# Gabrielcb/DaliID

Hardware: AMD Instinct MI355X
Metric: images/sec (train step) (higher is better)
Workload: dtype bf16; 1 GPU; configs[1]: ResNet-50 ReID bf16 256x128, PK batch 16x16=256 per GPU, center+proxy heads, Adam, EMA; global_batch=256, per_gpu_batch=256, parallelism=dp1

## Files before the change

### daliid_amd/csrc/conv.hip

```cpp
#include "gemm_tile.h"
#include "kernels.h"
#include "../../include/daliid_debug.h"
#include <cstdlib>
#include <type_traits>
#include <vector>
#include <string>
#include <cstdio>

namespace dali {

__device__ __forceinline__ void decode_pixel(const GatherGeom& g, int p, int& n, int& ho, int& wo) {
    if (g.lhw >= 0 && g.lw >= 0) {
        n = p >> g.lhw;
        const int rem = p & ((1 << g.lhw) - 1);
        ho = rem >> g.lw;
        wo = rem & ((1 << g.lw) - 1);
    } else {
        const int hw = g.Hout * g.Wout;
        n = p / hw;
        const int rem = p - n * hw;
        ho = rem / g.Wout;
        wo = rem - ho * g.Wout;
    }
}
// ... 1007 lines not shown
            for (int j = 0; j < FN; ++j) {
                const bf16x8_t fb = *reinterpret_cast<const bf16x8_t*>(patch + (boff[j] ^ (uint32_t)(h << 5)));
#pragma unroll
                for (int i = 0; i < FM; ++i) acc[i][j] = __builtin_amdgcn_mfma_f32_16x16x32_bf16(fa[i], fb, acc[i][j], 0, 0, 0);
            }
        }
        asm volatile("s_waitcnt lgkmcnt(0)" ::: "memory");
        __builtin_amdgcn_s_barrier();
    }
    conv_epilogue_g<TM, TN, FM, FN, 4, NT, EPI>(a, acc, 0, tn, smem, 0, wn);
}

}
#include "fused1x1.h"
namespace dali {

__device__ __forceinline__ int wg_swz(int row) { return (row & 3) | (((row >> 3) & 1) << 2); }

typedef short s16x4_t __attribute__((ext_vector_type(4)));

__device__ __forceinline__ int tr_frag_off(int chunk32, int lane, int half) {
    const int row = 8 * (lane >> 4) + ((lane & 15) >> 2) + 4 * half;
    return row * 128 + ((chunk32 ^ wg_swz(row)) << 4) + 4 * (lane & 3);
}
typedef short s16x8_t __attribute__((ext_vector_type(8)));
__device__ __forceinline__ bf16x8_t tr_frag(const uint16_t* tile, int chunk32, int lane) {
    typedef __attribute__((address_space(3))) s16x4_t* lds_ptr_t;
    const s16x4_t a = __builtin_amdgcn_ds_read_tr16_b64_v4i16((lds_ptr_t)(tile + tr_frag_off(chunk32, lane, 0)));
    const s16x4_t b = __builtin_amdgcn_ds_read_tr16_b64_v4i16((lds_ptr_t)(tile + tr_frag_off(chunk32, lane, 1)));
    return __builtin_bit_cast(bf16x8_t, s16x8_t{a[0], a[1], a[2], a[3], b[0], b[1], b[2], b[3]});
}

struct TrPair { s16x4_t lo, hi; };
__device__ __forceinline__ s16x4_t ds_read_tr_raw(const uint16_t* p) {
    typedef __attribute__((address_space(3))) const uint16_t* lds_cptr_t;
    const uint32_t addr = (uint32_t)(uintptr_t)(lds_cptr_t)p;
    s16x4_t v;
    asm volatile("ds_read_b64_tr_b16 %0, %1" : "=v"(v) : "v"(addr));
    return v;
}
__device__ __forceinline__ TrPair tr_frag_raw(const uint16_t* tile, int chunk32, int lane) {
    return TrPair{ds_read_tr_raw(tile + tr_frag_off(chunk32, lane, 0)), ds_read_tr_raw(tile + tr_frag_off(chunk32, lane, 1))};
}
__device__ __forceinline__ bf16x8_t tr_join(const TrPair& t) {
    return __builtin_bit_cast(bf16x8_t, s16x8_t{t.lo[0], t.lo[1], t.lo[2], t.lo[3], t.hi[0], t.hi[1], t.hi[2], t.hi[3]});
}
template <int N>
__device__ __forceinline__ void tr_settle(TrPair& a, TrPair& b, TrPair& c, TrPair& d) {
    static_assert(N == 0 || N == 8 || N == 10 || N == 16 || N == 18, "lgkmcnt immediates used by the callers");
    asm volatile("s_waitcnt lgkmcnt(%8)" : "+v"(a.lo), "+v"(a.hi), "+v"(b.lo), "+v"(b.hi), "+v"(c.lo), "+v"(c.hi), "+v"(d.lo), "+v"(d.hi) : "n"(N > 15 ? 15 : N));
}

__device__ __forceinline__ void tr_settle_all(TrPair& a) { asm volatile("s_waitcnt lgkmcnt(0)" : "+v"(a.lo), "+v"(a.hi)); }

template <int FM, int FN>
__device__ __forceinline__ void store_slab_tiles(float* slab, const f32x4_t (&acc)[FM][FN], int m_first, int n_first, int Cm, int Ntot, int lane) {
    const int mr = m_first + (lane >> 4) * 4, nc = n_first + (lane & 15);
    if (m_first + 16 * FM <= Cm && n_first + 16 * FN <= Ntot) {
        float* row = slab + (size_t)mr * Ntot + nc;
#pragma unroll
        for (int i = 0; i < FM; ++i)
#pragma unroll
            for (int rr = 0; rr < 4; ++rr) {
                float* p = row + (size_t)(i * 16 + rr) * Ntot;
#pragma unroll
                for (int j = 0; j < FN; ++j) p[j * 16] = acc[i][j][rr];
            }
        return;
    }
#pragma unroll
    for (int i = 0; i < FM; ++i)
#pragma unroll
        for (int j = 0; j < FN; ++j) {
            const int n = nc + j * 16;
#pragma unroll
            for (int rr = 0; rr < 4; ++rr) {
                const int m = mr + i * 16 + rr;
                if (m < Cm && n < Ntot) slab[(size_t)m * Ntot + n] = acc[i][j][rr];
            }
        }
}


struct WGradWork {
    int ks, tm, tn, p_begin, p_end, ksteps;
    __device__ __forceinline__ void set(const WGradArgs& a, unsigned item, int tiles_m, int tiles_n) {
        const unsigned tiles = tiles_m * tiles_n;
        ks = item / tiles;
        const int tile = item - ks * tiles;
        tm = tile / tiles_n; tn = tile - tm * tiles_n;
        p_begin = ks * a.pix_per_split;
        p_end = min(a.P, p_begin + a.pix_per_split);
        ksteps = (p_end > p_begin) ? (p_end - p_begin + 31) >> 5 : 0;
    }
    __device__ __forceinline__ bool map_xcd(const WGradArgs& a, int tiles_m, int tiles_n) {
        const int work = tiles_m * tiles_n * a.splits, per_xcd = (work + 7) >> 3;
        const int item = (blockIdx.x & 7) * per_xcd + (blockIdx.x >> 3);
        if ((int)(blockIdx.x >> 3) >= per_xcd || item >= work) return false;
        set(a, item, tiles_m, tiles_n);
        return true;
    }
};

struct WGradRsrc { __amdgpu_buffer_rsrc_t y, x; };
__device__ __forceinline__ WGradRsrc wgrad_rsrc(const WGradArgs& a) {
    const GatherGeom& g = a.g;
// ... 227 lines not shown
        }
    };

    f32x4_t acc[4][4];
#pragma unroll
    for (int i = 0; i < 4; ++i)
#pragma unroll
        for (int j = 0; j < 4; ++j) acc[i][j] = f32x4_t{0.f, 0.f, 0.f, 0.f};
    const bool do_cs = COLSUM && tn == 0 && wn == 0;
    f32x4_t cs[4];
#pragma unroll
    for (int i = 0; i < 4; ++i) cs[i] = f32x4_t{0.f, 0.f, 0.f, 0.f};
    typedef short ones_vec_t __attribute__((ext_vector_type(8)));
    const bf16x8_t ones = __builtin_bit_cast(bf16x8_t, ones_vec_t{0x3F80, 0x3F80, 0x3F80, 0x3F80, 0x3F80, 0x3F80, 0x3F80, 0x3F80});

    if (ksteps > 0) {
        issue(0, 0);
        if (ksteps > 1) issue(1, 1);
        if (ksteps > 1) dma_wait<4>(); else dma_wait<0>();
        __builtin_amdgcn_s_barrier();
        conv_stamp(a, 1);
        int st_cur = 0, st_nxt2 = 2;
        for (int kt = 0; kt < ksteps; ++kt) {
            if (kt + 2 < ksteps) issue(kt + 2, st_nxt2);
            const uint16_t* sa = smem + st_cur * 2 * TILE;
            const uint16_t* sb = sa + TILE;
            bf16x8_t fa[4];
            wgrad_tr_kstep(sa, wm * 4, sb, wn * 4, lane, acc, fa);
            if constexpr (COLSUM) if (do_cs) {
#pragma unroll
                for (int i = 0; i < 4; ++i) cs[i] = __builtin_amdgcn_mfma_f32_16x16x32_bf16(fa[i], ones, cs[i], 0, 0, 0);
            }
            if (kt + 2 < ksteps) dma_wait<4>(); else dma_wait<0>();
            __builtin_amdgcn_s_barrier();
            st_cur = (st_cur == 2) ? 0 : st_cur + 1;
            st_nxt2 = (st_nxt2 == 2) ? 0 : st_nxt2 + 1;
        }
    }
    conv_stamp(a, 2);
    float* slab = a.partial + (size_t)ks * a.Cm * a.Ntot;
    store_slab_tiles<4, 4>(slab, acc, m0 + wm * 64, n0 + wn * 64, a.Cm, a.Ntot, lane);
    if constexpr (COLSUM) if (do_cs && (lane & 15) == 0) {
#pragma unroll
        for (int i = 0; i < 4; ++i)
#pragma unroll
            for (int rr = 0; rr < 4; ++rr) {
                const int m = m0 + wm * 64 + i * 16 + (lane >> 4) * 4 + rr;
                if (m < a.Cm) a.colsum[(size_t)ks * a.Cm + m] = cs[i][rr];
            }
    }
    conv_stamp_stores(a);
}

__device__ __forceinline__ int halo_swz(int row) { return ((row >> 1) & 1) | (((row >> 3) & 1) << 1); }
constexpr int W3_A_ELEMS = 32 * 128, W3_B_ELEMS = 16 * 512, W3_STAGE = W3_A_ELEMS + W3_B_ELEMS;

template <int NSTAGE>
__global__ __launch_bounds__(512) void igemm_wgrad3x3_kernel(WGradArgs a, int tiles_m, int tiles_n) {
    extern __shared__ __attribute__((aligned(16))) uint16_t smem[];
    const int tid = threadIdx.x, lane = tid & 63;
    const int wave = __builtin_amdgcn_readfirstlane(tid >> 6);
    const int wm = wave >> 2, wn = wave & 3;
    WGradWork wk;
    if (!wk.map_xcd(a, tiles_m, tiles_n)) return;
    const int ks = wk.ks, m0 = wk.tm * 128, ci0 = wk.tn * 64;
    conv_stamp(a, 0);
    const bool m_active = m0 + wm * 64 < a.Cm;
    const GatherGeom g = a.g;
    const int W = g.Wout, H = g.Hout, Cin = g.Ck, lw = g.lw, lhw = g.lhw;
    const int RW = 32 >> lw, HC = W + 2, HP = (RW + 2) * HC;
    const WGradRsrc rs = wgrad_rsrc(a);

    const int r_in = lane >> 4, ps = lane & 15;
    const int c16 = ((((ps >> 1) ^ wg_swz(4 * wave + r_in)) << 1) | (ps & 1));
    const int am = m0 + c16 * 8;
    const bool a_ok = am < a.Cm;
    int hb_hr[2], hb_off[2];
    bool hb_ok[2];
#pragma unroll
    for (int i = 0; i < 2; ++i) {
        const int hp = 8 * (wave + 8 * i) + (lane >> 3);
        const int lc = (lane & 7) ^ (halo_swz(hp) << 1);
        const int hr = hp / HC, hc = hp - hr * HC;
        hb_hr[i] = hr;
        hb_ok[i] = hp < HP && (unsigned)(hc - 1) < (unsigned)W && ci0 + lc * 8 < Cin;
        hb_off[i] = ((hc - 1) * Cin + ci0 + lc * 8) * 2;
    }
    const int p_begin = wk.p_begin, p_end = wk.p_end, ksteps = wk.ksteps;

    auto issue = [&](int kt, int stage) {
        uint16_t* sa = smem + stage * W3_STAGE;
        uint16_t* sb = sa + W3_A_ELEMS;
        const int p0 = p_begin + kt * 32;
        const int p = p0 + 4 * wave + r_in;
        const uint32_t oa = (p < p_end && a_ok) ? (uint32_t)(p * a.Cm + am) * 2u : DMA_OOB;
        __builtin_amdgcn_raw_ptr_buffer_load_lds(rs.y, (lds_void_ptr)(sa + wave * 512), 16, oa, 0, 0, 0);
        const int n = p0 >> lhw, h_base = (p0 & ((1 << lhw) - 1)) >> lw;
        const int row_bytes = W * Cin * 2;
        const int img_base = (int)((long long)n * g.img_pitch * 2);
#pragma unroll
        for (int i = 0; i < 2; ++i) {
            const int h = h_base - 1 + hb_hr[i];
            const bool ok = hb_ok[i] && (unsigned)h < (unsigned)H && p0 < p_end;
            const uint32_t ob = ok ? (uint32_t)(img_base + h * row_bytes + hb_off[i]) : DMA_OOB;
            __builtin_amdgcn_raw_ptr_buffer_load_lds(rs.x, (lds_void_ptr)(sb + (wave + 8 * i) * 512), 16, ob, 0, 0, 0);
        }
    };

    f32x4_t acc[9][4];
#pragma unroll
    for (int t = 0; t < 9; ++t)
#pragma unroll
        for (int i = 0; i < 4; ++i) acc[t][i] = f32x4_t{0.f, 0.f, 0.f, 0.f};
    const int gq = lane >> 4, q = (lane & 15) >> 2, pp = lane & 3;
    const int hrow_base = ((8 * gq) >> lw) * HC + ((8 * gq) & (W - 1)) + q;
    int boff0[9], boff1[9];
#pragma unroll
    for (int r = 0; r < 3; ++r)
#pragma unroll
        for (int s2 = 0; s2 < 3; ++s2) {
            const int row0 = hrow_base + r * HC + s2, row1 = row0 + 4;
            boff0[r * 3 + s2] = row0 * 64 + ((wn ^ halo_swz(row0)) << 4) + 4 * pp;
            boff1[r * 3 + s2] = row1 * 64 + ((wn ^ halo_swz(row1)) << 4) + 4 * pp;
        }
    auto load_b = [&](const uint16_t* sb, int t) -> TrPair { return TrPair{ds_read_tr_raw(sb + boff0[t]), ds_read_tr_raw(sb + boff1[t])}; };

    constexpr int AHEAD = NSTAGE - 1;
    auto wait_inflight = [&](int n) {
        if (n <= 0) dma_wait<0>();
        else if (n == 1) dma_wait<3>();
        else if (n == 2) dma_wait<6>();
        else if (n == 3) dma_wait<9>();
        else dma_wait<12>();
    };
    static_assert(AHEAD >= 1 && AHEAD <= 5, "ring depth");
    if (ksteps > 0) {
        int issued = 0;
        for (; issued < AHEAD && issued < ksteps; ++issued) issue(issued, issued);
        wait_inflight(issued - 1 > 4 ? 4 : issued - 1);
        __builtin_amdgcn_s_barrier();
        conv_stamp(a, 1);
        int st_cur = 0, st_fill = AHEAD % NSTAGE;
        for (int kt = 0; kt < ksteps; ++kt) {
            if (kt + AHEAD < ksteps) issue(kt + AHEAD, st_fill);
            const uint16_t* sa = smem + st_cur * W3_STAGE;
            const uint16_t* sb = sa + W3_A_ELEMS;
            if (m_active) {
            TrPair ra[4], rb[9];
#pragma unroll
            for (int i = 0; i < 4; ++i) ra[i] = tr_frag_raw(sa, wm * 4 + i, lane);
#pragma unroll
            for (int t = 0; t < 9; ++t) rb[t] = load_b(sb, t);
            tr_settle<18>(ra[0], ra[1], ra[2], ra[3]);
            tr_settle<10>(rb[0], rb[1], rb[2], rb[3]);
            bf16x8_t fa[4];
#pragma unroll
            for (int i = 0; i < 4; ++i) fa[i] = tr_join(ra[i]);
#pragma unroll
            for (int t = 0; t < 4; ++t) {
                const bf16x8_t fb = tr_join(rb[t]);
#pragma unroll
                for (int i = 0; i < 4; ++i) acc[t][i] = __builtin_amdgcn_mfma_f32_16x16x32_bf16(fa[i], fb, acc[t][i], 0, 0, 0);
            }
            __builtin_amdgcn_sched_barrier(0);
            tr_settle<0>(rb[4], rb[5], rb[6], rb[7]);
            tr_settle_all(rb[8]);
#pragma unroll
            for (int t = 4; t < 9; ++t) {
                const bf16x8_t fb = tr_join(rb[t]);
#pragma unroll
                for (int i = 0; i < 4; ++i) acc[t][i] = __builtin_amdgcn_mfma_f32_16x16x32_bf16(fa[i], fb, acc[t][i], 0, 0, 0);
            }
            }
            const int left = ksteps - 1 - kt;
            const int keep = (left < AHEAD ? left : AHEAD) - 1;
            wait_inflight(keep > 4 ? 4 : keep);
            __builtin_amdgcn_s_barrier();
            st_cur = (st_cur == NSTAGE - 1) ? 0 : st_cur + 1;
            st_fill = (st_fill == NSTAGE - 1) ? 0 : st_fill + 1;
        }
    }
    conv_stamp(a, 2);
    float* slab = a.partial + (size_t)ks * a.Cm * a.Ntot;
    if (m_active) {
        float* row = slab + (size_t)(m0 + wm * 64 + (lane >> 4) * 4) * a.Ntot + ci0 + wn * 16 + (lane & 15);
#pragma unroll
        for (int i = 0; i < 4; ++i)
#pragma unroll
            for (int rr = 0; rr < 4; ++rr) {
                float* p = row + (size_t)(i * 16 + rr) * a.Ntot;
#pragma unroll
                for (int t = 0; t < 9; ++t) p[t * Cin] = acc[t][i][rr];
            }
    }
    conv_stamp_stores(a);
}

template <int WM, int WN, int NSTAGE, bool COLSUM = false>
__global__ __launch_bounds__(WM * WN * 64, 4) void igemm_wgrad_wg_kernel(WGradArgs a, int tiles_m, int tiles_n) {
    constexpr int TM = 64 * WM, TN = 64 * WN, NW = WM * WN;
    using Gather = WGradGather<TM / 128, (TM + TN) / 128, NW>;
    constexpr int IMG = Gather::IMG, NIMG_A = Gather::NIMG_A, STAGE = Gather::STAGE, NDMA = Gather::NDMA;
    constexpr int AHEAD = NSTAGE - 1;
    static_assert(TM % 128 == 0 && TN % 128 == 0, "unsupported wave grid");
    extern __shared__ __attribute__((aligned(16))) uint16_t smem[];
    const int tid = threadIdx.x, lane = tid & 63;
    const int wave = __builtin_amdgcn_readfirstlane(tid >> 6);
    const int wm = wave / WN, wn = wave % WN;
    WGradWork wk;
    if (!wk.map_xcd(a, tiles_m, tiles_n)) return;
    const int m0 = wk.tm * TM, n0 = wk.tn * TN, ksteps = wk.ksteps;
    const Gather gather(a, wave, m0, n0, wk.p_begin, wk.p_end, lane);

    const bool do_cs = COLSUM && wn == 0;
    int cs_turn = wk.tn;
    f32x4_t cs = f32x4_t{0.f, 0.f, 0.f, 0.f};
    typedef unsigned sel_vec_t __attribute__((ext_vector_type(4)));
    const int cs_col = (lane & 15) >> 2;
    f32x4_t acc[4][4];
#pragma unroll
    for (int i = 0; i < 4; ++i)
#pragma unroll
        for (int j = 0; j < 4; ++j) acc[i][j] = f32x4_t{0.f, 0.f, 0.f, 0.f};
    if (ksteps > 0) {
        int issued = 0;
        for (; issued < AHEAD && issued < ksteps; ++issued) gather.issue(issued, smem + issued * STAGE);
        if (issued == 1) dma_wait<0>();
        else if (issued == 2) dma_wait<NDMA>();
        else dma_wait<2 * NDMA>();
        __builtin_amdgcn_s_barrier();
        int st_cur = 0, st_fill = AHEAD % NSTAGE;
        for (int kt = 0; kt < ksteps; ++kt) {
            if (kt + AHEAD < ksteps) gather.issue(kt + AHEAD, smem + st_fill * STAGE);
            const uint16_t* sa = smem + st_cur * STAGE + (wm >> 1) * IMG;
            const uint16_t* sb = smem + st_cur * STAGE + (NIMG_A + (wn >> 1)) * IMG;
            bf16x8_t fa[4];
            wgrad_tr_kstep(sa, (wm & 1) * 4, sb, (wn & 1) * 4, lane, acc, fa);
            if constexpr (COLSUM) if (do_cs) {
                if (cs_turn == 0) {
                    int opaque;
// ... 374 lines not shown
    using Shape = RingShape<64, WM, WN, 4, 4, NSTAGE>;
    return {name, kfn(&igemm_conv_k64s_kernel<WM, WN, NP, NSTAGE, 4, 4, MODE, SRC2>), Shape::NT + NP * 64, Shape::LDS_BYTES, Shape::TM, Shape::TN, GRID_XCD};
}

static const GemmKernel
    CONV128_BN{"CONV128_BN", kfn(&igemm_conv_kernel<128, 128, true>), 256, REG128_LDS, 128, 128, GRID_XCD},
    CONV128{"CONV128", kfn(&igemm_conv_kernel<128, 128, false>), 256, REG128_LDS, 128, 128, GRID_XCD},
    DMA128 = ring_kernel<32, 2, 2, 4, 4, 3, 4, true, Epi::CONV>("DMA128"),
    DMA128_LIN = ring_kernel<32, 2, 2, 4, 4, 3, 4, true, Epi::LIN>("DMA128_LIN"),
    DMA128_FUSED = ring_kernel<32, 2, 2, 4, 4, 3, 3, true, Epi::FUSED>("DMA128_FUSED"),
    DMA128_CLS = ring_kernel<32, 2, 2, 4, 4, 3, 4, true, Epi::PARITY>("DMA128_CLS"),
    DMA128_SRC2 = ring_kernel<32, 2, 2, 4, 4, 3, 4, true, Epi::CONV, true>("DMA128_SRC2"),
    CONV64_BN{"CONV64_BN", kfn(&igemm_conv_kernel<64, 256, true>), 256, REG64_LDS, 64, 256, GRID_XCD},
    CONV64{"CONV64", kfn(&igemm_conv_kernel<64, 256, false>), 256, REG64_LDS, 64, 256, GRID_XCD},
    DMA64 = ring_kernel<32, 2, 2, 2, 8, 3, 2, true, Epi::GENERAL>("DMA64"),
    DMA64_LEAN = ring_kernel<32, 2, 2, 2, 8, 3, 2, true, Epi::FUSED_LEAN>("DMA64_LEAN"),
    DMA64_SRC2 = ring_kernel<32, 2, 2, 2, 8, 3, 2, true, Epi::GENERAL, true>("DMA64_SRC2"),
    K64S64 = k64s_kernel<1, 4, 4, 2, Epi::GENERAL>("K64S64"),
    HALO64{"HALO64", kfn(&igemm_conv_halo64_kernel<3, Epi::GENERAL>), 512, HALO64_LDS, 64, 256, GRID_HALO},
    HALO64_LEAN{"HALO64_LEAN", kfn(&igemm_conv_halo64_kernel<3, Epi::FUSED_LEAN>), 512, HALO64_LDS, 64, 256, GRID_HALO},
    WG128 = ring_kernel<32, 2, 4, 4, 4, 3, 4, false, Epi::CONV>("WG128"),
    WG128_LIN = ring_kernel<32, 2, 4, 4, 4, 3, 4, false, Epi::LIN>("WG128_LIN"),
    WG128_FUSED = ring_kernel<32, 2, 4, 4, 4, 3, 4, false, Epi::FUSED>("WG128_FUSED"),
    WG128_CLS = ring_kernel<32, 2, 4, 4, 4, 3, 4, false, Epi::PARITY>("WG128_CLS"),
    WG256 = ring_kernel<32, 4, 4, 4, 4, 4, 4, false, Epi::GENERAL>("WG256"),
    K64S = k64s_kernel<2, 4, 8, 3, Epi::CONV>("K64S"),
    K64S_LIN = k64s_kernel<2, 4, 8, 3, Epi::LIN>("K64S_LIN"),
    K64S_LEAN = k64s_kernel<2, 4, 8, 3, Epi::FUSED_LEAN>("K64S_LEAN"),
    K64S_SRC2 = k64s_kernel<2, 4, 8, 3, Epi::CONV, true>("K64S_SRC2"),
    K64 = ring_kernel<64, 4, 4, 4, 4, 2, 4, true, Epi::CONV>("K64"),
    K64_LIN = ring_kernel<64, 4, 4, 4, 4, 2, 4, true, Epi::LIN>("K64_LIN"),
    K64_FUSED = ring_kernel<64, 4, 4, 4, 4, 2, 4, true, Epi::FUSED>("K64_FUSED"),
    K64_CLS = ring_kernel<64, 4, 4, 4, 4, 2, 4, true, Epi::PARITY>("K64_CLS"),
    K64_SRC2 = ring_kernel<64, 4, 4, 4, 4, 2, 4, true, Epi::CONV, true>("K64_SRC2"),
    K64_FUSED_SRC2 = ring_kernel<64, 4, 4, 4, 4, 2, 4, true, Epi::FUSED, true>("K64_FUSED_SRC2"),
    K64_320 = ring_kernel<64, 4, 4, 4, 5, 2, 4, true, Epi::LIN>("K64_320");

template <int RB, bool RES, bool OM, bool BITS, bool SRC2 = false>
static GemmKernel f1_kernel() {
    static char name[32];
    snprintf(name, sizeof name, "F1_RB%d%s%s%s%s", RB, RES ? "_RES" : "", OM ? "_MASK" : "", BITS ? "_BITS" : "", SRC2 ? "_SRC2" : "");
    return {name, kfn(&fused1x1_persist_kernel<3, RB, RES, OM, BITS, SRC2>), (F1_NC + F1_NP + F1_NR) * 64, f1_lds_bytes(3, RB, RB == 2 ? 128 : F1_KMAX),
            F1_TM, F1_TN, GRID_CUS, 0, RB};
}
static const GemmKernel F1[2][2][2][2] = {
    {{{f1_kernel<2, false, false, false, true>(), f1_kernel<2, false, false, true>()}, {f1_kernel<2, false, true, false>(), f1_kernel<2, false, true, true>()}},
     {{f1_kernel<2, true, false, false>(), f1_kernel<2, true, false, true>()}, {f1_kernel<2, true, true, false>(), f1_kernel<2, true, true, true>()}}},
    {{{f1_kernel<1, false, false, false, true>(), f1_kernel<1, false, false, true>()}, {f1_kernel<1, false, true, false>(), f1_kernel<1, false, true, true>()}},
     {{f1_kernel<1, true, false, false>(), f1_kernel<1, true, false, true>()}, {f1_kernel<1, true, true, false>(), f1_kernel<1, true, true, true>()}}}};

static const GemmKernel
    WG_BN{"WG_BN", kfn(&igemm_wgrad_kernel<true>), 256, 0, 128, 128, GRID_SPLITS},
    WG_PLAIN{"WG_PLAIN", kfn(&igemm_wgrad_kernel<false>), 256, 0, 128, 128, GRID_SPLITS},
    WG_3X3{"WG_3X3", kfn(&igemm_wgrad3x3_kernel<3>), 512, 3 * W3_STAGE * 2, 128, 9 * 64, GRID_SPLITS8, 256};
static const GemmKernel WG_DMA[2] = {
    {"WG_DMA", kfn(&igemm_wgrad_dma_kernel<false>), 256, 0, 128, 128, GRID_SPLITS8},
    {"WG_DMA_COLSUM", kfn(&igemm_wgrad_dma_kernel<true>), 256, 0, 128, 128, GRID_SPLITS8}};
static const GemmKernel WG_WG[2] = {
    {"WG_WG", kfn(&igemm_wgrad_wg_kernel<2, 4, 3>), 512, ring_lds(128, 256, 32, 3), 128, 256, GRID_SPLITS8, 512},
    {"WG_WG_COLSUM", kfn(&igemm_wgrad_wg_kernel<2, 4, 3, true>), 512, ring_lds(128, 256, 32, 3), 128, 256, GRID_SPLITS8, 512}};
static const GemmKernel WG_P[2][2] = {
    {{"WG_P", kfn(&igemm_wgrad_p_kernel<2, 4, 4, 4, 8, 6>), 1024, ring_lds(128, 256, 32, 6), 128, 256, GRID_SPLITS8, 256},
     {"WG_P_COLSUM", kfn(&igemm_wgrad_p_kernel<2, 4, 4, 4, 8, 6, true>), 1024, ring_lds(128, 256, 32, 6), 128, 256, GRID_SPLITS8, 256}},
    {{"WG_P_FLAT", kfn(&igemm_wgrad_p_kernel<1, 4, 8, 4, 4, 6>), 512, ring_lds(128, 256, 32, 6), 128, 256, GRID_SPLITS8, 256},
     {"WG_P_FLAT_COLSUM", kfn(&igemm_wgrad_p_kernel<1, 4, 8, 4, 4, 6, true>), 512, ring_lds(128, 256, 32, 6), 128, 256, GRID_SPLITS8, 256}}};

struct GemmChoice {
    const GemmKernel* k = nullptr;
    int tiles_m = 0, tiles_n = 0, lds = 0, class_grid = 0;
    unsigned grid = 0;
    int rc = DALI_OK, why_arg = 0;
    const char* why = nullptr;
    GemmChoice() = default;
    GemmChoice(int rc_, const char* why_, int why_arg_ = 0) : rc(rc_), why_arg(why_arg_), why(why_) {}
    int refuse() const { set_error(why, why_arg); return rc; }
};
static GemmChoice gemm_place(const GemmKernel& k, int rows, int cols, int mult, int Ck) {
    GemmChoice c;
    c.k = &k;
    c.tiles_m = (rows + k.tm - 1) / k.tm;
    c.tiles_n = (cols + k.tn - 1) / k.tn;
    c.lds = k.f1_rb ? f1_lds_bytes(3, k.f1_rb, Ck) : k.lds;
    switch (k.grid) {
        case GRID_XCD: c.grid = xcd_tile_grid(c.tiles_m, c.tiles_n); break;
        case GRID_CLASSES: c.class_grid = xcd_tile_grid(c.tiles_m, c.tiles_n); c.grid = mult * c.class_grid; break;
        case GRID_CUS: c.grid = mult; break;
        case GRID_HALO: c.grid = c.tiles_n; break;
        case GRID_SPLITS: c.grid = c.tiles_m * c.tiles_n * mult; break;
        case GRID_SPLITS8: c.grid = (c.tiles_m * c.tiles_n * mult + 7) / 8 * 8; break;
    }
    return c;
}
template <class Args>
static int gemm_launch(hipStream_t st, const GemmChoice& c, Args& args) {
    const GemmKernel& k = *c.k;
    DeviceOnce::Guard once(k.once);
    if (k.lds > 64 * 1024 && once.first()) {
        DALI_HIP(hipFuncSetAttribute(k.fn, hipFuncAttributeMaxDynamicSharedMemorySize, k.lds));
        once.done();
    }
    int tiles_m = c.tiles_m, tiles_n = c.tiles_n;
    void* tile_args[] = {&args, &tiles_m, &tiles_n};
    void* halo_args[] = {&args, &tiles_n};
    (void)hipLaunchKernel(k.fn, dim3(c.grid), dim3(k.block), k.grid == GRID_HALO ? halo_args : tile_args, c.lds, st);
    DALI_LAUNCH_CHECK();
    return DALI_OK;
}
// ... 122 lines not shown
        return DALI_ERR_UNSUPPORTED;
    }
    if (c.k->grid == GRID_CLASSES) args.g.class_grid = c.class_grid;
    return gemm_launch(st, c, args);
}

template <class One>
static int conv_for_each_launch(const IGemmArgs& a, One&& one) {
    IGemmArgs args = a;
    GatherGeom& g = args.g;
    g.sub = 0; g.oph = g.opw = 0; g.Hfull = g.Hout; g.Wfull = g.Wout;
    g.r0 = 0; g.rstep = 1; g.nr = g.R; g.s0 = 0; g.sstep = 1; g.ns = g.S;
    if (g.mode == 1 && g.stride == 2 && conv_dma_ok(args) && !a.stats && (g.Hout % 2) == 0 && (g.Wout % 2) == 0 &&
        ilog2_exact(g.Wout / 2) >= 0 && ilog2_exact((g.Hout / 2) * (g.Wout / 2)) >= 0) {
        int nr[2], ns[2];
        for (int ph = 0; ph < 2; ++ph) {
            const int r0 = (ph + g.pad) & 1, s0 = (ph + g.pad) & 1;
            nr[ph] = r0 < g.R ? (g.R - r0 + 1) / 2 : 0;
            ns[ph] = s0 < g.S ? (g.S - s0 + 1) / 2 : 0;
        }
        const bool all_have = nr[0] && nr[1] && ns[0] && ns[1];
        if (all_have && a.Cm > 64 && (a.Cm & 7) == 0) {
            IGemmArgs s = args;
            s.g.sub = 2; s.g.oph = s.g.opw = 0; s.g.Hfull = g.Hout; s.g.Wfull = g.Wout;
            s.g.Hout = g.Hout / 2; s.g.Wout = g.Wout / 2; s.P = a.P / 4;
            s.g.r0 = s.g.s0 = 0; s.g.rstep = s.g.sstep = 2;
            s.g.nr = nr[0] > nr[1] ? nr[0] : nr[1]; s.g.ns = ns[0] > ns[1] ? ns[0] : ns[1];
            return one(s);
        }
        if (all_have || (a.Res != nullptr && a.Res == a.O)) {
            for (int ph = 0; ph < 2; ++ph)
                for (int pw = 0; pw < 2; ++pw) {
                    if (nr[ph] * ns[pw] == 0) continue;
                    IGemmArgs s = args;
                    s.g.sub = 1; s.g.oph = ph; s.g.opw = pw; s.g.Hfull = g.Hout; s.g.Wfull = g.Wout;
                    s.g.Hout = g.Hout / 2; s.g.Wout = g.Wout / 2; s.P = a.P / 4;
                    s.g.r0 = (ph + g.pad) & 1; s.g.rstep = 2; s.g.nr = nr[ph];
                    s.g.s0 = (pw + g.pad) & 1; s.g.sstep = 2; s.g.ns = ns[pw];
                    const int rc = one(s);
                    if (rc) return rc;
                }
            return DALI_OK;
        }
    }
    return one(args);
}
int launch_igemm_conv(hipStream_t st, const IGemmArgs& a) {
    IGemmArgs args = a;
    args.stamps = g_conv_stamps;
    return conv_for_each_launch(args, [&](const IGemmArgs& s) { return launch_igemm_conv_one(st, s); });
}

static bool wgrad_spec(int Cm, int Ntot) { return ((Cm + 127) / 128) * ((Ntot + 255) / 256) <= 100; }
static int wgrad_pick_cfg(int Cm, int Ntot, int taps, int P, int halo_w) {
    if (taps == 9 && (halo_w == 8 || halo_w == 16 || halo_w == 32) && Cm % 64 == 0 && (Ntot / 9) % 64 == 0 && P % 32 == 0) return 3;
    if (taps == 7 && Ntot == 224 && P >= 16384) return 2;
    return (taps == 1 && Ntot >= 256 && P >= 16384) ? 2 : 0;
}
static const GemmKernel& wgrad_kernel(int cfg, int Cm, int Ntot, bool in_bn, bool dma_ok, bool colsum, bool flat) {
    if (in_bn) return WG_BN;
    if (!dma_ok) return WG_PLAIN;
    if (cfg == 3) return WG_3X3;
    if (cfg == 2) return wgrad_spec(Cm, Ntot) ? WG_P[flat][colsum] : WG_WG[colsum];
    return WG_DMA[colsum];
}
static bool wgrad_colsum_ok(int cfg, bool in_bn, bool dma_ok) { return cfg != 3 && !in_bn && dma_ok; }
static int colsum_rows_of(const GemmKernel& k, int Ntot, int splits) { return k.tn == 128 ? splits : splits * ((Ntot + k.tn - 1) / k.tn); }

static void wgrad_plan(int Cm, int Ntot, int P, int target_blocks, int* splits, int* pix_per_split, int taps, int halo_w) {
    const GemmKernel& k = wgrad_kernel(wgrad_pick_cfg(Cm, Ntot, taps, P, halo_w), Cm, Ntot, false, true, false, true);
    if (k.plan_wgs) target_blocks = k.plan_wgs;
    const int tiles = ((Cm + k.tm - 1) / k.tm) * ((Ntot + k.tn - 1) / k.tn);
    int sp = (target_blocks + tiles - 1) / tiles;
    const int max_sp = (P + 255) / 256;
    if (sp > max_sp) sp = max_sp;
    if (sp < 1) sp = 1;
    {
        int best = sp;
        double best_cost = (double)((tiles * sp + target_blocks - 1) / target_blocks) / sp;
        for (int c = sp - 1; c >= 1 && c >= sp / 2; --c) {
            const double cost = (double)((tiles * c + target_blocks - 1) / target_blocks) / c;
            if (cost <= best_cost + 1e-12) { best = c; best_cost = cost; }
        }
        sp = best;
    }
    int pps = ((P + sp - 1) / sp + 31) & ~31;
    sp = (P + pps - 1) / pps;
    *splits = sp; *pix_per_split = pps;
}

static int wgrad_halo_w(const GatherGeom& g, bool in_bn) {
    const bool halo = !in_bn && g.R == 3 && g.S == 3 && g.stride == 1 && g.pad == 1 && g.mode == 0 && ilog2_exact(g.Wout) >= 0 &&
                      ilog2_exact(g.Hout * g.Wout) >= 7 && g.Hin == g.Hout && g.Win == g.Wout && g.pix_pitch == g.Ck && g.row_pitch == g.Win * g.Ck;
    return halo ? g.Wout : 0;
}

struct WGradChoice { int Ntot, splits, pix_per_split, colsum_rows; GemmChoice c; };
static WGradChoice wgrad_choose(int Cm, int P, const GatherGeom& g, bool in_bn, bool want_colsum) {
    WGradChoice w{};
    const int taps = g.R * g.S, halo_w = wgrad_halo_w(g, in_bn);
    w.Ntot = taps * g.Ck;
    wgrad_plan(Cm, w.Ntot, P, 512, &w.splits, &w.pix_per_split, taps, halo_w);
    const int cfg = wgrad_pick_cfg(Cm, w.Ntot, taps, P, halo_w);
    const bool dma_ok = gather_dma_ok(g, P, (long long)P * Cm * 2);
    const bool colsum = want_colsum && wgrad_colsum_ok(cfg, in_bn, dma_ok);
    w.c = gemm_place(wgrad_kernel(cfg, Cm, w.Ntot, in_bn, dma_ok, colsum, plain_rows(g)), Cm, w.Ntot, w.splits, g.Ck);
    w.colsum_rows = colsum ? colsum_rows_of(*w.c.k, w.Ntot, w.splits) : 0;
    return w;
}

WGradNeed wgrad_need(int Cm, int P, const GatherGeom& g, bool colsum, bool operand_transform) {
    const WGradChoice w = wgrad_choose(Cm, P, g, operand_transform, colsum);
    return WGradNeed{(size_t)w.splits * Cm * w.Ntot * sizeof(float), colsum ? std::max((size_t)w.colsum_rows * Cm, colsum_partial_floats(P, Cm)) : 0};
}

int launch_wgrad(hipStream_t st, WGradArgs a, const WGradBufs& ws, float* out, int accumulate, float* colsum_out) {
    const WGradChoice w = wgrad_choose(a.Cm, a.P, a.g, a.in_scale != nullptr, colsum_out != nullptr);
    a.Ntot = w.Ntot; a.splits = w.splits; a.pix_per_split = w.pix_per_split;
    a.partial = ws.slab;
// ... 82 lines not shown
            set_error("gemm_profile_end: event query failed"); rc = DALI_ERR_HIP; break;
        }
        total_ms[p->cls[i]] += ms; total_flops[p->cls[i]] += p->flops[i]; launches[p->cls[i]] += 1;
        if (dump) fprintf(dump, "%zu,%s,us=%.2f,gflop=%.3f\n", i, p->desc[i].c_str(), ms * 1e3, p->flops[i] * 1e-9);
    }
    if (dump) fclose(dump);
    for (auto& e : p->ev) (void)hipEventDestroy(e);
    delete p;
    return rc;
}

static int fill_geom(GatherGeom& g, int n_img, int Hin, int Win, int Ck, int Hout, int Wout, int R, int S, int stride, int pad, int mode) {
    g.Hout = Hout; g.Wout = Wout; g.Hin = Hin; g.Win = Win; g.Ck = Ck; g.R = R; g.S = S; g.stride = stride; g.pad = pad;
    g.mode = mode;
    g.pix_pitch = Ck; g.row_pitch = Win * Ck; g.img_pitch = (long long)Hin * Win * Ck;
    g.lw = g.lhw = -1;
    (void)n_img;
    return 0;
}

extern "C" int dali_debug_conv_kernel_name(int Cm, int P, int h, int wd, int ck, int r, int s, int stride, int pad, int mode, int flags, int ck1, int x_rep,
                                           int n_cus, char* out, int cap) {
    DALI_REQUIRE(out && cap > 0 && Cm > 0 && P > 0 && ck > 0 && (mode == 0 || mode == 1) && (stride == 1 || stride == 2), "dali_debug_conv_kernel_name: bad argument");
    static char here[4];
    const auto stand_in = [&](int bit, int i) { return (flags & bit) ? here + i : nullptr; };
    IGemmArgs a{};
    a.W = reinterpret_cast<const uint16_t*>(here); a.X = a.W; a.O = reinterpret_cast<uint16_t*>(here + 1);
    a.Cm = Cm; a.P = P;
    if (mode == 0) fill_geom(a.g, 0, h, wd, ck, (h + 2 * pad - r) / stride + 1, (wd + 2 * pad - s) / stride + 1, r, s, stride, pad, 0);
    else fill_geom(a.g, 0, (h + 2 * pad - r) / stride + 1, (wd + 2 * pad - s) / stride + 1, ck, h, wd, r, s, stride, pad, 1);
    a.stats = reinterpret_cast<float*>(stand_in(DALI_DEBUG_CONV_STATS, 2));
    a.Res = reinterpret_cast<const uint16_t*>(stand_in(DALI_DEBUG_CONV_RES, 2));
    a.res_mask = reinterpret_cast<const uint8_t*>(stand_in(DALI_DEBUG_CONV_RES_MASK, 2));
    a.out_mask = reinterpret_cast<const uint8_t*>(stand_in(DALI_DEBUG_CONV_OUT_MASK, 2));
    a.bits_out = reinterpret_cast<uint8_t*>(stand_in(DALI_DEBUG_CONV_BITS, 2));
    a.out_scale = a.out_shift = reinterpret_cast<const float*>(stand_in(DALI_DEBUG_CONV_FUSED, 2));
    a.out_relu = (flags & DALI_DEBUG_CONV_FUSED) ? 1 : 0;
    a.act = (flags & DALI_DEBUG_CONV_LIN) ? 1 : 0;
    if (ck1 > 0) { a.X2 = a.X; a.Ck1 = ck1; a.x_rep = x_rep; }
    std::string names;
    const int rc = conv_for_each_launch(a, [&](const IGemmArgs& one) {
        const GemmChoice c = conv_choose(one, n_cus);
        if (!c.k) return c.refuse();
        names += names.empty() ? "" : "+";
        names += c.k->name;
        return (int)DALI_OK;
    });
    if (rc) return rc;
    DALI_REQUIRE((int)names.size() < cap, "dali_debug_conv_kernel_name: the name takes %d bytes", (int)names.size() + 1);
    snprintf(out, (size_t)cap, "%s", names.c_str());
    return DALI_OK;
}

extern "C" int dali_conv2d_fwd(dali_ctx* ctx, void* stream, const uint16_t* x, const uint16_t* w, uint16_t* y,
                               int n, int h, int wd, int cin, int cout, int r, int s, int stride, int pad,
                               const float* in_scale, const float* in_shift, int in_relu, float* stats) {
    DALI_REQUIRE(ctx && x && w && y, "dali_conv2d_fwd: null argument");
    DALI_REQUIRE(cin % 32 == 0 && cout % 4 == 0, "dali_conv2d_fwd: cin must be a multiple of 32 and cout of 4 (cin=%d cout=%d)", cin, cout);
    DALI_REQUIRE(stride == 1 || stride == 2, "dali_conv2d_fwd: stride %d unsupported", stride);
    DALI_REQUIRE((in_scale == nullptr) == (in_shift == nullptr), "dali_conv2d_fwd: in_scale/in_shift must come together");
    const int ho = (h + 2 * pad - r) / stride + 1, wo = (wd + 2 * pad - s) / stride + 1;
    IGemmArgs a{};
    a.W = w; a.X = x; a.O = y; a.Res = nullptr; a.in_scale = in_scale; a.in_shift = in_shift; a.stats = stats;
    a.Cm = cout; a.P = n * ho * wo; a.in_relu = in_relu;
    fill_geom(a.g, n, h, wd, cin, ho, wo, r, s, stride, pad, 0);
    return launch_igemm_conv((hipStream_t)stream, a);
}

extern "C" int dali_conv2d_bn_act(dali_ctx* ctx, void* stream, const uint16_t* x, const uint16_t* w, uint16_t* y, int n, int h, int wd, int cin, int cout,
                                  int r, int s, int stride, int pad, const float* out_scale, const float* out_shift, int out_relu) {
    DALI_REQUIRE(ctx && x && w && y && out_scale && out_shift, "dali_conv2d_bn_act: null argument");
    DALI_REQUIRE(cin % 32 == 0 && cout % 8 == 0, "dali_conv2d_bn_act: cin must be a multiple of 32 and cout of 8 (cin=%d cout=%d)", cin, cout);
    DALI_REQUIRE(stride == 1 || stride == 2, "dali_conv2d_bn_act: stride %d unsupported", stride);
    const int ho = (h + 2 * pad - r) / stride + 1, wo = (wd + 2 * pad - s) / stride + 1;
    IGemmArgs a{};
    a.W = w; a.X = x; a.O = y;
    a.out_scale = out_scale; a.out_shift = out_shift; a.out_relu = out_relu;
    a.Cm = cout; a.P = n * ho * wo;
    fill_geom(a.g, n, h, wd, cin, ho, wo, r, s, stride, pad, 0);
    return launch_igemm_conv((hipStream_t)stream, a);
}

extern "C" int dali_conv2d_stat_tiles(int cout, int cin, int r, int s, int stride, int pad, int n, int ho, int wo, int fused_operand) {
    (void)stride; (void)pad;
    return igemm_conv_stat_tiles(cout, n * ho * wo, r * s * cin, fused_operand != 0);
}

extern "C" int dali_conv2d_dgrad(dali_ctx* ctx, void* stream, const uint16_t* dy, const uint16_t* wt, uint16_t* dx,
                                 const uint16_t* residual, const uint8_t* residual_mask, int n, int h, int wd, int cin, int cout, int r, int s,
                                 int stride, int pad) {
    DALI_REQUIRE(ctx && dy && wt && dx, "dali_conv2d_dgrad: null argument");
    DALI_REQUIRE(!residual_mask || (residual && cin % 8 == 0), "dali_conv2d_dgrad: residual_mask needs a residual and cin %% 8 == 0 (cin=%d)", cin);
    DALI_REQUIRE(cout % 32 == 0 && cin % 4 == 0, "dali_conv2d_dgrad: cout must be a multiple of 32 and cin of 4 (cin=%d cout=%d)", cin, cout);
    DALI_REQUIRE(stride == 1 || stride == 2, "dali_conv2d_dgrad: stride %d unsupported", stride);
    const int ho = (h + 2 * pad - r) / stride + 1, wo = (wd + 2 * pad - s) / stride + 1;
    IGemmArgs a{};
    a.W = wt; a.X = dy; a.O = dx; a.Res = residual; a.res_mask = residual_mask; a.in_scale = nullptr; a.in_shift = nullptr; a.stats = nullptr;
    a.Cm = cin; a.P = n * h * wd; a.in_relu = 0;
    fill_geom(a.g, n, ho, wo, cout, h, wd, r, s, stride, pad, 1);
    return launch_igemm_conv((hipStream_t)stream, a);
}

extern "C" int dali_conv2d_wgrad(dali_ctx* ctx, void* stream, const uint16_t* x, const uint16_t* dy, float* dw,
                                 int n, int h, int wd, int cin, int cout, int r, int s, int stride, int pad,
                                 const float* in_scale, const float* in_shift, int in_relu, int accumulate) {
    DALI_REQUIRE(ctx && x && dy && dw, "dali_conv2d_wgrad: null argument");
// ... 108 lines not shown
```

### include/daliid_debug.h

```cpp
#ifndef DALIID_DEBUG_H
#define DALIID_DEBUG_H

#include <stdint.h>

#ifdef __cplusplus
extern "C" {
#endif

int dali_debug_reload_env(void);

int dali_debug_set_conv_stamps(void* dev_ptr);

int dali_debug_wgrad_splits(int Cm, int Ntot, int P, int taps, int halo_w);

enum {
    DALI_DEBUG_CONV_STATS = 1,
    DALI_DEBUG_CONV_FUSED = 2,
    DALI_DEBUG_CONV_RES = 4,
    DALI_DEBUG_CONV_RES_MASK = 8,
    DALI_DEBUG_CONV_OUT_MASK = 16,
    DALI_DEBUG_CONV_BITS = 32,
    DALI_DEBUG_CONV_LIN = 64
};
int dali_debug_conv_kernel_name(int Cm, int P, int h, int wd, int ck, int r, int s, int stride, int pad, int mode, int flags, int ck1, int x_rep,
                                int n_cus, char* out, int cap);

int dali_debug_splitk_reduce(void* stream, const float* partial, float* out, long long elems, int splits, int accumulate);

struct dali_resnet;
int dali_debug_resnet_backward_block(struct dali_resnet* net, void* stream, const float* d_emb, int block);

struct dali_vit;
int dali_debug_vit_backward_block(struct dali_vit* net, void* stream, const float* d_feat, int block);
int dali_debug_vit_tensor(const struct dali_vit* net, const char* name, void** ptr, int64_t* bytes);

struct dali_ctx;
int dali_debug_stem_wgrad(struct dali_ctx* ctx, void* stream, const float* images, const unsigned short* d_raw0, int N, int H, int W, int Cout, float* dw);
int dali_debug_head_pool_bwd_masked(struct dali_ctx* ctx, void* stream, const float* df, const short* arg, int n, int hw, int C, int mode,
                                    const unsigned char* ybits, unsigned short* dx);

#ifdef __cplusplus
}
#endif
#endif
```

Measured before the change: 17220 images/s.

## Add narrow 32-channel tile variant of 3x3 weight-gradient kernel for small layers

Templates the 3x3 wgrad kernel on the input-channel tile width and adds a 32-wide variant with a 4-stage ring, 2 M-fragments per wave, a different halo swizzle and a pipelined B-fragment load schedule. The variant is chosen for layers with Cm*Ck <= 256*256 (e.g. 64/128-channel ResNet layers), which yields more tiles and higher occupancy (launch bound of 4 blocks) where the 64-wide tile underfills the GPU. The cost is less reuse of A per tile and more halo traffic. Debug hooks are added to force a tile width and query the chosen kernel.

Result: no change. 17210 images/s (-0.0%).

```diff
diff --git a/daliid_amd/csrc/conv.hip b/daliid_amd/csrc/conv.hip
--- a/daliid_amd/csrc/conv.hip
+++ b/daliid_amd/csrc/conv.hip
@@ -1083,6 +1083,8 @@
 }
 
 __device__ __forceinline__ void tr_settle_all(TrPair& a) { asm volatile("s_waitcnt lgkmcnt(0)" : "+v"(a.lo), "+v"(a.hi)); }
+template <int N>
+__device__ __forceinline__ void tr_settle2(TrPair& a, TrPair& b) { asm volatile("s_waitcnt lgkmcnt(%4)" : "+v"(a.lo), "+v"(a.hi), "+v"(b.lo), "+v"(b.hi) : "n"(N)); }
 
 template <int FM, int FN>
 __device__ __forceinline__ void store_slab_tiles(float* slab, const f32x4_t (&acc)[FM][FN], int m_first, int n_first, int Cm, int Ntot, int lane) {
@@ -1416,20 +1418,31 @@
     conv_stamp_stores(a);
 }
 
-__device__ __forceinline__ int halo_swz(int row) { return ((row >> 1) & 1) | (((row >> 3) & 1) << 1); }
-constexpr int W3_A_ELEMS = 32 * 128, W3_B_ELEMS = 16 * 512, W3_STAGE = W3_A_ELEMS + W3_B_ELEMS;
-
-template <int NSTAGE>
-__global__ __launch_bounds__(512) void igemm_wgrad3x3_kernel(WGradArgs a, int tiles_m, int tiles_n) {
+template <int CI>
+__device__ __forceinline__ int halo_swz(int row) {
+    static_assert(CI == 64 || CI == 32, "halo row of 128 or 64 bytes");
+    return CI == 64 ? ((row >> 1) & 1) | (((row >> 3) & 1) << 1) : (row >> 3) & 1;
+}
+constexpr int W3_A_ELEMS = 32 * 128;
+constexpr int w3_b_elems(int ci_tile) { return 128 * ci_tile; }
+constexpr int w3_stage(int ci_tile) { return W3_A_ELEMS + w3_b_elems(ci_tile); }
+constexpr int w3_lds(int ci_tile, int stages) { return stages * w3_stage(ci_tile) * 2; }
+
+template <int NSTAGE, int CI>
+__global__ __launch_bounds__(512, CI == 64 ? 2 : 4) void igemm_wgrad3x3_kernel(WGradArgs a, int tiles_m, int tiles_n) {
+    constexpr int WN = CI / 16, WM = 8 / WN, FM = 8 / WM;
+    constexpr int W3_STAGE = w3_stage(CI);
+    constexpr int LPP = CI / 8, PXP = 64 / LPP;
+    constexpr int NHB = 128 / PXP / 8;
     extern __shared__ __attribute__((aligned(16))) uint16_t smem[];
     const int tid = threadIdx.x, lane = tid & 63;
     const int wave = __builtin_amdgcn_readfirstlane(tid >> 6);
-    const int wm = wave >> 2, wn = wave & 3;
+    const int wm = wave / WN, wn = wave % WN;
     WGradWork wk;
     if (!wk.map_xcd(a, tiles_m, tiles_n)) return;
-    const int ks = wk.ks, m0 = wk.tm * 128, ci0 = wk.tn * 64;
+    const int ks = wk.ks, m0 = wk.tm * 128, ci0 = wk.tn * CI;
     conv_stamp(a, 0);
-    const bool m_active = m0 + wm * 64 < a.Cm;
+    const bool m_active = m0 + wm * 16 * FM < a.Cm;
     const GatherGeom g = a.g;
     const int W = g.Wout, H = g.Hout, Cin = g.Ck, lw = g.lw, lhw = g.lhw;
     const int RW = 32 >> lw, HC = W + 2, HP = (RW + 2) * HC;
@@ -1439,12 +1452,12 @@
     const int c16 = ((((ps >> 1) ^ wg_swz(4 * wave + r_in)) << 1) | (ps & 1));
     const int am = m0 + c16 * 8;
     const bool a_ok = am < a.Cm;
-    int hb_hr[2], hb_off[2];
-    bool hb_ok[2];
-#pragma unroll
-    for (int i = 0; i < 2; ++i) {
-        const int hp = 8 * (wave + 8 * i) + (lane >> 3);
-        const int lc = (lane & 7) ^ (halo_swz(hp) << 1);
+    int hb_hr[NHB], hb_off[NHB];
+    bool hb_ok[NHB];
+#pragma unroll
+    for (int i = 0; i < NHB; ++i) {
+        const int hp = PXP * (wave + 8 * i) + lane / LPP;
+        const int lc = (lane % LPP) ^ (halo_swz<CI>(hp) << 1);
         const int hr = hp / HC, hc = hp - hr * HC;
         hb_hr[i] = hr;
         hb_ok[i] = hp < HP && (unsigned)(hc - 1) < (unsigned)W && ci0 + lc * 8 < Cin;
@@ -1463,7 +1476,7 @@
         const int row_bytes = W * Cin * 2;
         const int img_base = (int)((long long)n * g.img_pitch * 2);
 #pragma unroll
-        for (int i = 0; i < 2; ++i) {
+        for (int i = 0; i < NHB; ++i) {
             const int h = h_base - 1 + hb_hr[i];
             const bool ok = hb_ok[i] && (unsigned)h < (unsigned)H && p0 < p_end;
             const uint32_t ob = ok ? (uint32_t)(img_base + h * row_bytes + hb_off[i]) : DMA_OOB;
@@ -1471,11 +1484,11 @@
         }
     };
 
-    f32x4_t acc[9][4];
+    f32x4_t acc[9][FM];
 #pragma unroll
     for (int t = 0; t < 9; ++t)
 #pragma unroll
-        for (int i = 0; i < 4; ++i) acc[t][i] = f32x4_t{0.f, 0.f, 0.f, 0.f};
+        for (int i = 0; i < FM; ++i) acc[t][i] = f32x4_t{0.f, 0.f, 0.f, 0.f};
     const int gq = lane >> 4, q = (lane & 15) >> 2, pp = lane & 3;
     const int hrow_base = ((8 * gq) >> lw) * HC + ((8 * gq) & (W - 1)) + q;
     int boff0[9], boff1[9];
@@ -1484,18 +1497,19 @@
 #pragma unroll
         for (int s2 = 0; s2 < 3; ++s2) {
             const int row0 = hrow_base + r * HC + s2, row1 = row0 + 4;
-            boff0[r * 3 + s2] = row0 * 64 + ((wn ^ halo_swz(row0)) << 4) + 4 * pp;
-            boff1[r * 3 + s2] = row1 * 64 + ((wn ^ halo_swz(row1)) << 4) + 4 * pp;
+            boff0[r * 3 + s2] = row0 * CI + ((wn ^ halo_swz<CI>(row0)) << 4) + 4 * pp;
+            boff1[r * 3 + s2] = row1 * CI + ((wn ^ halo_swz<CI>(row1)) << 4) + 4 * pp;
+            if constexpr (CI == 32) asm volatile("" : "+v"(boff0[r * 3 + s2]), "+v"(boff1[r * 3 + s2]));
         }
     auto load_b = [&](const uint16_t* sb, int t) -> TrPair { return TrPair{ds_read_tr_raw(sb + boff0[t]), ds_read_tr_raw(sb + boff1[t])}; };
 
-    constexpr int AHEAD = NSTAGE - 1;
+    constexpr int AHEAD = NSTAGE - 1, NDMA = 1 + NHB;
     auto wait_inflight = [&](int n) {
         if (n <= 0) dma_wait<0>();
-        else if (n == 1) dma_wait<3>();
-        else if (n == 2) dma_wait<6>();
-        else if (n == 3) dma_wait<9>();
-        else dma_wait<12>();
+        else if (n == 1) dma_wait<NDMA>();
+        else if (n == 2) dma_wait<2 * NDMA>();
+        else if (n == 3) dma_wait<3 * NDMA>();
+        else dma_wait<4 * NDMA>();
     };
     static_assert(AHEAD >= 1 && AHEAD <= 5, "ring depth");
     if (ksteps > 0) {
@@ -1509,7 +1523,38 @@
             if (kt + AHEAD < ksteps) issue(kt + AHEAD, st_fill);
             const uint16_t* sa = smem + st_cur * W3_STAGE;
             const uint16_t* sb = sa + W3_A_ELEMS;
+            if constexpr (CI == 32) {
             if (m_active) {
+            TrPair ra[FM], rb[2][2];
+#pragma unroll
+            for (int i = 0; i < FM; ++i) ra[i] = tr_frag_raw(sa, wm * FM + i, lane);
+            rb[0][0] = load_b(sb, 0); rb[0][1] = load_b(sb, 1);
+            bf16x8_t fa[FM];
+#pragma unroll
+            for (int b = 0; b < 5; ++b) {
+                if (b < 4) {
+                    rb[(b + 1) & 1][0] = load_b(sb, 2 * b + 2);
+                    if (b < 3) rb[(b + 1) & 1][1] = load_b(sb, 2 * b + 3);
+                }
+                if (b == 0) {
+                    static_assert(FM == 2, "A fragments of the narrow tile");
+                    tr_settle2<4>(ra[0], ra[1]);
+#pragma unroll
+                    for (int i = 0; i < FM; ++i) fa[i] = tr_join(ra[i]);
+                }
+                if (b < 3) tr_settle2<4>(rb[b & 1][0], rb[b & 1][1]);
+                else if (b == 3) tr_settle2<2>(rb[1][0], rb[1][1]);
+                else tr_settle_all(rb[0][0]);
+#pragma unroll
+                for (int j = 0; j < (b < 4 ? 2 : 1); ++j) {
+                    const bf16x8_t fb = tr_join(rb[b & 1][j]);
+#pragma unroll
+                    for (int i = 0; i < FM; ++i) acc[2 * b + j][i] = __builtin_amdgcn_mfma_f32_16x16x32_bf16(fa[i], fb, acc[2 * b + j][i], 0, 0, 0);
+                }
+                __builtin_amdgcn_sched_barrier(0);
+            }
+            }
+            } else if (m_active) {
             TrPair ra[4], rb[9];
 #pragma unroll
             for (int i = 0; i < 4; ++i) ra[i] = tr_frag_raw(sa, wm * 4 + i, lane);
@@ -1547,9 +1592,9 @@
     conv_stamp(a, 2);
     float* slab = a.partial + (size_t)ks * a.Cm * a.Ntot;
     if (m_active) {
-        float* row = slab + (size_t)(m0 + wm * 64 + (lane >> 4) * 4) * a.Ntot + ci0 + wn * 16 + (lane & 15);
-#pragma unroll
-        for (int i = 0; i < 4; ++i)
+        float* row = slab + (size_t)(m0 + wm * 16 * FM + (lane >> 4) * 4) * a.Ntot + ci0 + wn * 16 + (lane & 15);
+#pragma unroll
+        for (int i = 0; i < FM; ++i)
 #pragma unroll
             for (int rr = 0; rr < 4; ++rr) {
                 float* p = row + (size_t)(i * 16 + rr) * a.Ntot;
@@ -2030,7 +2075,8 @@
 static const GemmKernel
     WG_BN{"WG_BN", kfn(&igemm_wgrad_kernel<true>), 256, 0, 128, 128, GRID_SPLITS},
     WG_PLAIN{"WG_PLAIN", kfn(&igemm_wgrad_kernel<false>), 256, 0, 128, 128, GRID_SPLITS},
-    WG_3X3{"WG_3X3", kfn(&igemm_wgrad3x3_kernel<3>), 512, 3 * W3_STAGE * 2, 128, 9 * 64, GRID_SPLITS8, 256};
+    WG_3X3{"WG_3X3", kfn(&igemm_wgrad3x3_kernel<3, 64>), 512, w3_lds(64, 3), 128, 9 * 64, GRID_SPLITS8, 256},
+    WG_3X3_N32{"WG_3X3_N32", kfn(&igemm_wgrad3x3_kernel<4, 32>), 512, w3_lds(32, 4), 128, 9 * 32, GRID_SPLITS8, 512};
 static const GemmKernel WG_DMA[2] = {
     {"WG_DMA", kfn(&igemm_wgrad_dma_kernel<false>), 256, 0, 128, 128, GRID_SPLITS8},
     {"WG_DMA_COLSUM", kfn(&igemm_wgrad_dma_kernel<true>), 256, 0, 128, 128, GRID_SPLITS8}};
@@ -2259,8 +2305,15 @@
 }
 
 static bool wgrad_spec(int Cm, int Ntot) { return ((Cm + 127) / 128) * ((Ntot + 255) / 256) <= 100; }
+static int g_wgrad3x3_tile = 0;
+static bool wgrad3x3_narrow(int Cm, int Ck, int P) {
+    if (g_wgrad3x3_tile) return g_wgrad3x3_tile == 32;
+    (void)P;
+    return Cm % 128 == 0 && Cm * Ck <= 256 * 256;
+}
 static int wgrad_pick_cfg(int Cm, int Ntot, int taps, int P, int halo_w) {
-    if (taps == 9 && (halo_w == 8 || halo_w == 16 || halo_w == 32) && Cm % 64 == 0 && (Ntot / 9) % 64 == 0 && P % 32 == 0) return 3;
+    if (taps == 9 && (halo_w == 8 || halo_w == 16 || halo_w == 32) && Cm % 64 == 0 && (Ntot / 9) % 64 == 0 && P % 32 == 0)
+        return wgrad3x3_narrow(Cm, Ntot / 9, P) ? 4 : 3;
     if (taps == 7 && Ntot == 224 && P >= 16384) return 2;
     return (taps == 1 && Ntot >= 256 && P >= 16384) ? 2 : 0;
 }
@@ -2268,10 +2321,11 @@
     if (in_bn) return WG_BN;
     if (!dma_ok) return WG_PLAIN;
     if (cfg == 3) return WG_3X3;
+    if (cfg == 4) return WG_3X3_N32;
     if (cfg == 2) return wgrad_spec(Cm, Ntot) ? WG_P[flat][colsum] : WG_WG[colsum];
     return WG_DMA[colsum];
 }
-static bool wgrad_colsum_ok(int cfg, bool in_bn, bool dma_ok) { return cfg != 3 && !in_bn && dma_ok; }
+static bool wgrad_colsum_ok(int cfg, bool in_bn, bool dma_ok) { return cfg != 3 && cfg != 4 && !in_bn && dma_ok; }
 static int colsum_rows_of(const GemmKernel& k, int Ntot, int splits) { return k.tn == 128 ? splits : splits * ((Ntot + k.tn - 1) / k.tn); }
 
 static void wgrad_plan(int Cm, int Ntot, int P, int target_blocks, int* splits, int* pix_per_split, int taps, int halo_w) {
@@ -2460,6 +2514,26 @@
     return DALI_OK;
 }
 
+extern "C" int dali_debug_wgrad_kernel_name(int Cm, int n, int h, int wd, int ck, int r, int s, int stride, int pad, int* splits, int* pix_per_split, char* out,
+                                            int cap) {
+    DALI_REQUIRE(out && cap > 0 && Cm > 0 && n > 0 && ck > 0 && (stride == 1 || stride == 2), "dali_debug_wgrad_kernel_name: bad argument");
+    GatherGeom g{};
+    const int ho = (h + 2 * pad - r) / stride + 1, wo = (wd + 2 * pad - s) / stride + 1;
+    fill_geom(g, n, h, wd, ck, ho, wo, r, s, stride, pad, 0);
+    const WGradChoice w = wgrad_choose(Cm, n * ho * wo, g, false, false);
+    const std::string name = w.c.k->name;
+    DALI_REQUIRE((int)name.size() < cap, "dali_debug_wgrad_kernel_name: the name takes %d bytes", (int)name.size() + 1);
+    snprintf(out, (size_t)cap, "%s", name.c_str());
+    if (splits) *splits = w.splits;
+    if (pix_per_split) *pix_per_split = w.pix_per_split;
+    return DALI_OK;
+}
+extern "C" int dali_debug_wgrad3x3_tile(int ci_tile) {
+    DALI_REQUIRE(ci_tile == 0 || ci_tile == 32 || ci_tile == 64, "dali_debug_wgrad3x3_tile: 0 (by shape), 32 or 64, not %d", ci_tile);
+    g_wgrad3x3_tile = ci_tile;
+    return DALI_OK;
+}
+
 extern "C" int dali_conv2d_fwd(dali_ctx* ctx, void* stream, const uint16_t* x, const uint16_t* w, uint16_t* y,
                                int n, int h, int wd, int cin, int cout, int r, int s, int stride, int pad,
                                const float* in_scale, const float* in_shift, int in_relu, float* stats) {
diff --git a/include/daliid_debug.h b/include/daliid_debug.h
--- a/include/daliid_debug.h
+++ b/include/daliid_debug.h
@@ -25,6 +25,10 @@
 int dali_debug_conv_kernel_name(int Cm, int P, int h, int wd, int ck, int r, int s, int stride, int pad, int mode, int flags, int ck1, int x_rep,
                                 int n_cus, char* out, int cap);
 
+int dali_debug_wgrad_kernel_name(int Cm, int n, int h, int wd, int ck, int r, int s, int stride, int pad, int* splits, int* pix_per_split, char* out,
+                                 int cap);
+int dali_debug_wgrad3x3_tile(int ci_tile);
+
 int dali_debug_splitk_reduce(void* stream, const float* partial, float* out, long long elems, int splits, int accumulate);
 
 struct dali_resnet;
```
